# taldatech/soft-intro-vae-pytorch

Hardware: AMD Instinct MI355X
Metric: training images/sec (whole node) at 256x256 bs128 (higher is better)
Workload: dtype f32; 1 GPU; soft_intro_vae celeb256 256x256 zdim=512 channels=[64, 128, 256, 512, 512, 512], full E-step + D-step iteration; global_batch=128, per_gpu_batch=128, parallelism=dp1, decoder_forward_reuse=True, hip_graph=False, batchnorm=local

## Files before the change

### soft-intro-vae-pytorch_amd/csrc/bn.hip

```cpp
#include "common.h"

namespace {

struct SlicePlan {
  int S;
  long long len;
};
static SlicePlan plan_slices(long long n_per_ch, int C) {
  SlicePlan p;
  long long s1 = (n_per_ch + 8191) / 8192;
  long long s2 = 2048 / C;
  if (s2 < 1) s2 = 1;
  long long S = s1 < s2 ? s1 : s2;
  if (S < 1) S = 1;
  long long len = (n_per_ch + S - 1) / S;
  len = (len + 3) & ~3LL;
  p.S = (int)((n_per_ch + len - 1) / len);
  p.len = len;
  return p;
}

}

__device__ __forceinline__ unsigned sign_nibble(const float4 v) {
// ... 54 lines not shown
                                                         float* __restrict__ mean_out,
                                                         float* __restrict__ invstd_out) {
  const int c = blockIdx.x * 64 + threadIdx.x;
  if (c == 0 && num_batches_tracked) *num_batches_tracked += 1;
  if (c >= C) return;
  double sum = 0.0, sq = 0.0;
  for (int s = 0; s < S; ++s) {
    const size_t o = ((size_t)c * S + s) * 2;
    sum += part[o];
    sq += part[o + 1];
  }
  const double mean = sum / count;
  double var = sq / count - mean * mean;
  if (var < 0.0) var = 0.0;
  const float invstd = (float)(1.0 / sqrt(var + (double)eps));
  mean_out[c] = (float)mean;
  invstd_out[c] = invstd;
  if (running_mean) {
    const double unbiased = count > 1.0 ? var * count / (count - 1.0) : var;
    running_mean[c] = (float)((1.0 - momentum) * running_mean[c] + momentum * mean);
    running_var[c] = (float)((1.0 - momentum) * running_var[c] + momentum * unbiased);
  }
}

template <int NT>
__global__ void __launch_bounds__(NT) bn_finalize_conv_kernel(const float* __restrict__ part, int S, int C,
                                                               double count, float eps, float momentum,
                                                               float* running_mean, float* running_var,
                                                               long long* num_batches_tracked,
                                                               float* __restrict__ mean_out,
                                                               float* __restrict__ invstd_out, int nseg, int seg_rev) {
  __shared__ double red[NT / 64];
  const int c = blockIdx.x;
  for (int gi = 0; gi < nseg; ++gi) {
    const int g = seg_rev ? nseg - 1 - gi : gi;
    double sum = 0.0, sq = 0.0;
    for (int s = threadIdx.x; s < S; s += NT) {
      const float2 v = *reinterpret_cast<const float2*>(part + ((size_t)(g * S + s) * C + c) * 2);
      sum += (double)v.x;
      sq += (double)v.y;
    }
    sum = block_sum<NT>(sum, red);
    sq = block_sum<NT>(sq, red);
    if (threadIdx.x == 0) {
      if (c == 0 && num_batches_tracked) *num_batches_tracked += 1;
      const double mean = sum / count;
      double var = sq / count - mean * mean;
      if (var < 0.0) var = 0.0;
      mean_out[g * C + c] = (float)mean;
      invstd_out[g * C + c] = (float)(1.0 / sqrt(var + (double)eps));
      if (running_mean) {
        const double unbiased = count > 1.0 ? var * count / (count - 1.0) : var;
        running_mean[c] = (float)((1.0 - momentum) * running_mean[c] + momentum * mean);
        running_var[c] = (float)((1.0 - momentum) * running_var[c] + momentum * unbiased);
      }
    }
    __syncthreads();
  }
}

extern "C" size_t sivae_bn_workspace_bytes(int B, int C, int HW) {
  if (B <= 0 || C <= 0 || HW <= 0) return 0;
  SlicePlan p = plan_slices((long long)B * HW, C);
  return ((size_t)C * p.S * 2 + (size_t)C * 2) * sizeof(double);
}

extern "C" int sivae_bn_stats(const float* x, int B, int C, int HW, float eps, float momentum,
                              float* running_mean, float* running_var, long long* num_batches_tracked,
                              float* mean_out, float* invstd_out, void* workspace, size_t workspace_bytes,
                              hipStream_t stream) {
  if (!x || !mean_out || !invstd_out) return SIVAE_ERR_NULL;
  if ((running_mean == nullptr) != (running_var == nullptr)) return SIVAE_ERR_NULL;
  if (B <= 0 || C <= 0 || HW <= 0) return SIVAE_ERR_SHAPE;
  if (!workspace || workspace_bytes < sivae_bn_workspace_bytes(B, C, HW)) return SIVAE_ERR_WORKSPACE;
  const long long n = (long long)B * HW;
  SlicePlan p = plan_slices(n, C);
  double* part = (double*)workspace;
  hipLaunchKernelGGL(bn_stats_partial_kernel, dim3(C, p.S), dim3(256), 0, stream, x, part, C, HW, n, p.len, p.S);
  hipLaunchKernelGGL(bn_finalize_kernel, dim3(cdiv(C, 64)), dim3(64), 0, stream, (const double*)part, p.S, C,
                     (double)n, eps, momentum, running_mean, running_var, num_batches_tracked, mean_out,
                     invstd_out);
  return sivae_launch_status();
}

static int bn_stats_from_conv_impl(const float* partials, int n_tiles, int nseg, int seg_rev, int B, int C, int HW,
                                   float eps, float momentum, float* running_mean, float* running_var,
                                   long long* num_batches_tracked, float* mean_out, float* invstd_out,
                                   hipStream_t stream) {
  if (!partials || !mean_out || !invstd_out) return SIVAE_ERR_NULL;
  if ((running_mean == nullptr) != (running_var == nullptr)) return SIVAE_ERR_NULL;
  if (B <= 0 || C <= 0 || HW <= 0 || n_tiles <= 0 || nseg <= 0 || (n_tiles % nseg) != 0) return SIVAE_ERR_SHAPE;
  const int S = n_tiles / nseg;
  if (S >= 4096)
    hipLaunchKernelGGL((bn_finalize_conv_kernel<1024>), dim3(C), dim3(1024), 0, stream, partials, S, C,
                       (double)B * HW, eps, momentum, running_mean, running_var, num_batches_tracked, mean_out,
                       invstd_out, nseg, seg_rev);
  else
    hipLaunchKernelGGL((bn_finalize_conv_kernel<256>), dim3(C), dim3(256), 0, stream, partials, S, C,
                       (double)B * HW, eps, momentum, running_mean, running_var, num_batches_tracked, mean_out,
                       invstd_out, nseg, seg_rev);
  return sivae_launch_status();
}

#define BNC_ROWS 128
__global__ void __launch_bounds__(256) bn_conv_rows_partial_kernel(const float* __restrict__ part, int S, int C,
                                                                   int nchunks, double* __restrict__ out) {
  __shared__ double red[2][256];
  const int chunk = blockIdx.x, g = blockIdx.y, t = threadIdx.x;
  int cw = 1;
  while (cw < C && cw < 256) cw <<= 1;
  const int rp = 256 / cw, tx = t & (cw - 1), ty = t / cw;
  const int r0 = chunk * BNC_ROWS;
  const int r1 = r0 + BNC_ROWS < S ? r0 + BNC_ROWS : S;
  for (int c0 = 0; c0 < C; c0 += cw) {
    const int c = c0 + tx;
    double sum = 0.0, sq = 0.0;
    if (c < C)
      for (int r = r0 + ty; r < r1; r += rp) {
        const float2 v = *reinterpret_cast<const float2*>(part + ((size_t)(g * S + r) * C + c) * 2);
        sum += (double)v.x;
        sq += (double)v.y;
      }
    red[0][t] = sum;
    red[1][t] = sq;
    __syncthreads();
    if (ty == 0 && c < C) {
      double a = 0.0, b = 0.0;
      for (int k = 0; k < rp; ++k) {
        a += red[0][k * cw + tx];
        b += red[1][k * cw + tx];
      }
      double* o = out + (((size_t)g * C + c) * nchunks + chunk) * 2;
      o[0] = a;
      o[1] = b;
    }
    __syncthreads();
  }
}

__global__ void __launch_bounds__(64) bn_conv_rows_finalize_kernel(const double* __restrict__ part2, int nchunks, int C,
                                                                   double count, float eps, float momentum,
                                                                   float* running_mean, float* running_var,
                                                                   long long* num_batches_tracked,
                                                                   float* __restrict__ mean_out,
                                                                   float* __restrict__ invstd_out, int nseg,
                                                                   int seg_rev) {
  const int c = blockIdx.x, lane = threadIdx.x;
  if (c == 0 && lane == 0 && num_batches_tracked) *num_batches_tracked += nseg;
  for (int gi = 0; gi < nseg; ++gi) {
    const int g = seg_rev ? nseg - 1 - gi : gi;
    const double* p = part2 + ((size_t)g * C + c) * nchunks * 2;
    double sum = 0.0, sq = 0.0;
    for (int k = lane; k < nchunks; k += 64) {
      sum += p[2 * k];
      sq += p[2 * k + 1];
    }
    sum = wave_sum(sum);
    sq = wave_sum(sq);
    if (lane == 0) {
      const double mean = sum / count;
      double var = sq / count - mean * mean;
      if (var < 0.0) var = 0.0;
      mean_out[g * C + c] = (float)mean;
      invstd_out[g * C + c] = (float)(1.0 / sqrt(var + (double)eps));
      if (running_mean) {
        const double unbiased = count > 1.0 ? var * count / (count - 1.0) : var;
        running_mean[c] = (float)((1.0 - momentum) * running_mean[c] + momentum * mean);
        running_var[c] = (float)((1.0 - momentum) * running_var[c] + momentum * unbiased);
      }
    }
  }
}

extern "C" size_t sivae_bn_stats_from_conv_workspace_bytes(int n_tiles, int nseg, int C) {
  if (n_tiles <= 0 || nseg <= 0 || C <= 0 || (n_tiles % nseg) != 0) return 0;
  const int S = n_tiles / nseg;
  if (S < 2048) return 0;
  return (size_t)nseg * C * cdiv(S, BNC_ROWS) * 2 * sizeof(double);
}

extern "C" int sivae_bn_stats_from_conv_ws(const float* partials, int n_tiles, int nseg, int seg_rev, int B_seg, int C,
                                           int HW, float eps, float momentum, float* running_mean, float* running_var,
                                           long long* num_batches_tracked, float* mean_out, float* invstd_out,
                                           void* workspace, size_t workspace_bytes, hipStream_t stream) {
  const size_t need = sivae_bn_stats_from_conv_workspace_bytes(n_tiles, nseg, C);
  if (need == 0)
    return bn_stats_from_conv_impl(partials, n_tiles, nseg, seg_rev, B_seg, C, HW, eps, momentum, running_mean,
                                   running_var, num_batches_tracked, mean_out, invstd_out, stream);
  if (!partials || !mean_out || !invstd_out) return SIVAE_ERR_NULL;
  if ((running_mean == nullptr) != (running_var == nullptr)) return SIVAE_ERR_NULL;
  if (B_seg <= 0 || HW <= 0) return SIVAE_ERR_SHAPE;
  if (!workspace || workspace_bytes < need) return SIVAE_ERR_WORKSPACE;
  const int S = n_tiles / nseg, nchunks = cdiv(S, BNC_ROWS);
  double* part2 = (double*)workspace;
  hipLaunchKernelGGL(bn_conv_rows_partial_kernel, dim3(nchunks, nseg), dim3(256), 0, stream, partials, S, C, nchunks,
                     part2);
  hipLaunchKernelGGL(bn_conv_rows_finalize_kernel, dim3(C), dim3(64), 0, stream, (const double*)part2, nchunks,
                     C, (double)B_seg * HW, eps, momentum, running_mean, running_var, num_batches_tracked, mean_out,
                     invstd_out, nseg, seg_rev);
  return sivae_launch_status();
}

extern "C" int sivae_bn_stats_from_conv_seg(const float* partials, int n_tiles, int nseg, int seg_rev, int B_seg, int C,
                                            int HW, float eps, float momentum, float* running_mean, float* running_var,
                                            long long* num_batches_tracked, float* mean_out, float* invstd_out,
                                            hipStream_t stream) {
  return bn_stats_from_conv_impl(partials, n_tiles, nseg, seg_rev, B_seg, C, HW, eps, momentum, running_mean,
                                 running_var, num_batches_tracked, mean_out, invstd_out, stream);
}

__global__ void __launch_bounds__(256) bn_sums_conv_kernel(const float* __restrict__ part, int S, int C,
                                                           double* __restrict__ sums) {
  __shared__ double red[4];
  const int c = blockIdx.x;
  double sum = 0.0, sq = 0.0;
  for (int s = threadIdx.x; s < S; s += 256) {
    const float2 v = *reinterpret_cast<const float2*>(part + ((size_t)s * C + c) * 2);
    sum += (double)v.x;
    sq += (double)v.y;
  }
  sum = block_sum<256>(sum, red);
  sq = block_sum<256>(sq, red);
  if (threadIdx.x == 0) {
    sums[c * 2 + 0] = sum;
    sums[c * 2 + 1] = sq;
  }
}

__global__ void __launch_bounds__(64) bn_finalize_sums_kernel(const double* __restrict__ sums, int C, double count,
                                                              float eps, float momentum, float* running_mean,
                                                              float* running_var, long long* num_batches_tracked,
                                                              float* __restrict__ mean_out,
                                                              float* __restrict__ invstd_out) {
  const int c = blockIdx.x * 64 + threadIdx.x;
  if (c >= C) return;
  if (c == 0 && num_batches_tracked) *num_batches_tracked += 1;
  const double mean = sums[c * 2] / count;
  double var = sums[c * 2 + 1] / count - mean * mean;
  if (var < 0.0) var = 0.0;
  mean_out[c] = (float)mean;
  invstd_out[c] = (float)(1.0 / sqrt(var + (double)eps));
  if (running_mean) {
    const double unbiased = count > 1.0 ? var * count / (count - 1.0) : var;
    running_mean[c] = (float)((1.0 - momentum) * running_mean[c] + momentum * mean);
    running_var[c] = (float)((1.0 - momentum) * running_var[c] + momentum * unbiased);
  }
}

extern "C" int sivae_bn_sums_from_conv(const float* partials, int n_tiles, int C, double* sums, hipStream_t stream) {
  if (!partials || !sums) return SIVAE_ERR_NULL;
  if (C <= 0 || n_tiles <= 0) return SIVAE_ERR_SHAPE;
  hipLaunchKernelGGL(bn_sums_conv_kernel, dim3(C), dim3(256), 0, stream, partials, n_tiles, C, sums);
  return sivae_launch_status();
}

extern "C" int sivae_bn_finalize_sums(const double* sums, int C, double count, float eps, float momentum,
                                      float* running_mean, float* running_var, long long* num_batches_tracked,
                                      float* mean_out, float* invstd_out, hipStream_t stream) {
  if (!sums || !mean_out || !invstd_out) return SIVAE_ERR_NULL;
  if ((running_mean == nullptr) != (running_var == nullptr)) return SIVAE_ERR_NULL;
  if (C <= 0 || !(count > 0.0)) return SIVAE_ERR_SHAPE;
  hipLaunchKernelGGL(bn_finalize_sums_kernel, dim3(cdiv(C, 64)), dim3(64), 0, stream, sums, C, count, eps, momentum,
                     running_mean, running_var, num_batches_tracked, mean_out, invstd_out);
  return sivae_launch_status();
}

__global__ void __launch_bounds__(64) bn_update_running_seg_kernel(const float* __restrict__ mean,
                                                                   const float* __restrict__ invstd, int nseg,
                                                                   int seg_rev, int C, double count, float eps,
                                                                   float momentum, float* running_mean,
                                                                   float* running_var, long long* num_batches_tracked) {
  const int c = blockIdx.x * 64 + threadIdx.x;
  if (c == 0 && num_batches_tracked) *num_batches_tracked += nseg;
  if (c >= C) return;
  float rm = running_mean[c], rv = running_var[c];
  for (int gi = 0; gi < nseg; ++gi) {
    const int g = seg_rev ? nseg - 1 - gi : gi;
    const double is = (double)invstd[g * C + c];
    double var = 1.0 / (is * is) - (double)eps;
    if (var < 0.0) var = 0.0;
    const double unbiased = count > 1.0 ? var * count / (count - 1.0) : var;
    rm = (float)((1.0 - momentum) * rm + momentum * (double)mean[g * C + c]);
    rv = (float)((1.0 - momentum) * rv + momentum * unbiased);
  }
  running_mean[c] = rm;
  running_var[c] = rv;
}

extern "C" int sivae_bn_update_running_seg(const float* mean, const float* invstd, int nseg, int seg_rev, int C,
                                           double count, float eps, float momentum, float* running_mean,
                                           float* running_var, long long* num_batches_tracked, hipStream_t stream) {
  if (!mean || !invstd || !running_mean || !running_var) return SIVAE_ERR_NULL;
  if (C <= 0 || nseg <= 0 || count <= 0.0) return SIVAE_ERR_SHAPE;
  hipLaunchKernelGGL(bn_update_running_seg_kernel, dim3(cdiv(C, 64)), dim3(64), 0, stream, mean, invstd, nseg, seg_rev,
                     C, count, eps, momentum, running_mean, running_var, num_batches_tracked);
  return sivae_launch_status();
}

static bool normalise_segments(int B, int& segB) {
  if (segB < 0 || (segB > 0 && B % segB != 0)) return false;
  if (segB == B) segB = 0;
  return true;
}

template <bool HAS_RES, bool VEC>
__global__ void __launch_bounds__(256) bn_apply_kernel(const float* __restrict__ x, const float* __restrict__ res,
                                                       const float* __restrict__ mean,
                                                       const float* __restrict__ invstd,
                                                       const float* __restrict__ gamma,
                                                       const float* __restrict__ beta, float slope,
                                                       float* __restrict__ y, unsigned char* __restrict__ mask,
                                                       int C, int HW, size_t numel, int segB) {
  const size_t stride = (size_t)gridDim.x * 256;
  if (VEC) {
    const size_t n4 = numel >> 2;
    for (size_t base = (size_t)blockIdx.x * 256; base < n4; base += stride) {
      const size_t i = base + threadIdx.x;
      const bool ok = i < n4;
      unsigned nib = 0;
      if (ok) {
        const size_t e = i << 2;
        const unsigned pl = (unsigned)(e / HW);
        const int c = (int)(pl % (unsigned)C);
        const int sc = segB > 0 ? c + (int)((pl / (unsigned)C) / (unsigned)segB) * C : c;
        const float m = mean[sc], g = invstd[sc] * gamma[c], bt = beta[c];
        float4 v = reinterpret_cast<const float4*>(x)[i];
        v.x = (v.x - m) * g + bt;
        v.y = (v.y - m) * g + bt;
        v.z = (v.z - m) * g + bt;
        v.w = (v.w - m) * g + bt;
        if (HAS_RES) {
          const float4 r = reinterpret_cast<const float4*>(res)[i];
          v.x += r.x; v.y += r.y; v.z += r.z; v.w += r.w;
        }
        nib = sign_nibble(v);
        v.x = lrelu(v.x, slope); v.y = lrelu(v.y, slope); v.z = lrelu(v.z, slope); v.w = lrelu(v.w, slope);
        reinterpret_cast<float4*>(y)[i] = v;
      }
      if (mask != nullptr) {
        const unsigned byte = pair_nibbles(nib);
        if (ok && !(threadIdx.x & 1)) mask[i >> 1] = (unsigned char)byte;
      }
    }
  } else {
    for (size_t e = (size_t)blockIdx.x * 256 + threadIdx.x; e < numel; e += stride) {
      const unsigned pl = (unsigned)(e / HW);
      const int c = (int)(pl % (unsigned)C);
      const int sc = segB > 0 ? c + (int)((pl / (unsigned)C) / (unsigned)segB) * C : c;
      float v = (x[e] - mean[sc]) * (invstd[sc] * gamma[c]) + beta[c];
      if (HAS_RES) v += res[e];
      y[e] = lrelu(v, slope);
    }
  }
}

static int bn_apply_impl(const float* x, const float* res, const float* mean, const float* invstd,
                         const float* gamma, const float* beta, float slope, float* y, unsigned char* mask, int B,
                         int C, int HW, hipStream_t stream, int segB) {
  if (!x || !mean || !invstd || !gamma || !beta || !y) return SIVAE_ERR_NULL;
  if (B <= 0 || C <= 0 || HW <= 0) return SIVAE_ERR_SHAPE;
  if (!normalise_segments(B, segB)) return SIVAE_ERR_SHAPE;
  const size_t numel = (size_t)B * C * HW;
  const bool vec = (HW & 3) == 0;
  if (mask && !vec) return SIVAE_ERR_SHAPE;
  long long work = vec ? (long long)(numel >> 2) : (long long)numel;
  int nb = cdiv(work, 256);
  if (nb > 8192) nb = 8192;
  if (nb < 1) nb = 1;
#define LAUNCH(R, V) \
  hipLaunchKernelGGL((bn_apply_kernel<R, V>), dim3(nb), dim3(256), 0, stream, x, res, mean, invstd, gamma, beta, \
                     slope, y, mask, C, HW, numel, segB)
  if (res) {
    if (vec) LAUNCH(true, true); else LAUNCH(true, false);
  } else {
    if (vec) LAUNCH(false, true); else LAUNCH(false, false);
  }
#undef LAUNCH
  return sivae_launch_status();
}

__global__ void __launch_bounds__(256) bn_apply_resup_kernel(const float* __restrict__ x, const float* __restrict__ res,
                                                             const float* __restrict__ mean,
                                                             const float* __restrict__ invstd,
                                                             const float* __restrict__ gamma,
                                                             const float* __restrict__ beta, float slope,
                                                             float* __restrict__ y, unsigned char* __restrict__ mask,
                                                             int C, int H, int W, size_t numel, int segB) {
  const size_t stride = (size_t)gridDim.x * 256;
  const int W4 = W >> 2, Hs = H >> 1, Ws = W >> 1;
  const size_t n4 = numel >> 2;
  for (size_t base = (size_t)blockIdx.x * 256; base < n4; base += stride) {
    const size_t i = base + threadIdx.x;
    const bool ok = i < n4;
    unsigned nib = 0;
    if (ok) {
      const int w4 = (int)(i % W4);
      size_t t = i / W4;
      const int h = (int)(t % H);
      t /= H;
      const int c = (int)(t % C);
      const int sc = segB > 0 ? c + (int)(((unsigned)t / (unsigned)C) / (unsigned)segB) * C : c;
      const float m = mean[sc], g = invstd[sc] * gamma[c], bt = beta[c];
      float4 v = reinterpret_cast<const float4*>(x)[i];
      const float2 r = *reinterpret_cast<const float2*>(res + (t * Hs + (h >> 1)) * Ws + 2 * w4);
      v.x = (v.x - m) * g + bt + r.x;
      v.y = (v.y - m) * g + bt + r.x;
      v.z = (v.z - m) * g + bt + r.y;
      v.w = (v.w - m) * g + bt + r.y;
      nib = sign_nibble(v);
      v.x = lrelu(v.x, slope); v.y = lrelu(v.y, slope); v.z = lrelu(v.z, slope); v.w = lrelu(v.w, slope);
      reinterpret_cast<float4*>(y)[i] = v;
    }
    if (mask != nullptr) {
      const unsigned byte = pair_nibbles(nib);
      if (ok && !(threadIdx.x & 1)) mask[i >> 1] = (unsigned char)byte;
    }
  }
}

static int bn_apply_resup_impl(const float* x, const float* res_half, const float* mean, const float* invstd,
                               const float* gamma, const float* beta, float slope, float* y, unsigned char* mask,
                               int B, int C, int H, int W, hipStream_t stream, int segB) {
  if (!x || !res_half || !mean || !invstd || !gamma || !beta || !y) return SIVAE_ERR_NULL;
  if (B <= 0 || C <= 0 || H <= 0 || W <= 0 || (H & 1) || (W & 3)) return SIVAE_ERR_SHAPE;
  if (!normalise_segments(B, segB)) return SIVAE_ERR_SHAPE;
  const size_t numel = (size_t)B * C * H * W;
  int nb = cdiv((long long)(numel >> 2), 256 * 4);
  if (nb > 8192) nb = 8192;
  if (nb < 1) nb = 1;
  hipLaunchKernelGGL(bn_apply_resup_kernel, dim3(nb), dim3(256), 0, stream, x, res_half, mean, invstd, gamma, beta,
                     slope, y, mask, C, H, W, numel, segB);
  return sivae_launch_status();
}

template <bool HAS_RES>
__global__ void __launch_bounds__(256) bn_apply_pool_kernel(const float* __restrict__ x, const float* __restrict__ res,
                                                            const float* __restrict__ mean,
                                                            const float* __restrict__ invstd,
                                                            const float* __restrict__ gamma,
                                                            const float* __restrict__ beta, float slope,
                                                            float* __restrict__ y, float* __restrict__ yp,
                                                            unsigned char* __restrict__ mask, int C, int H, int W,
                                                            size_t n_quads, int segB) {
  const size_t stride = (size_t)gridDim.x * 256;
  const int W4 = W >> 2, H2 = H >> 1;
  for (size_t base = (size_t)blockIdx.x * 256; base < n_quads; base += stride) {
    const size_t i = base + threadIdx.x;
    const bool ok = i < n_quads;
    unsigned nib0 = 0, nib1 = 0;
    size_t m0 = 0, m1 = 0;
    if (ok) {
      const int w4 = (int)(i % W4);
      size_t t = i / W4;
      const int h2 = (int)(t % H2);
      t /= H2;
      const int c = (int)(t % C);
      const int sc = segB > 0 ? c + (int)(((unsigned)t / (unsigned)C) / (unsigned)segB) * C : c;
      const float m = mean[sc], g = invstd[sc] * gamma[c], bt = beta[c];
      const size_t o0 = (t * H + 2 * h2) * (size_t)W + 4 * w4, o1 = o0 + W;
      float4 a = *reinterpret_cast<const float4*>(x + o0), b = *reinterpret_cast<const float4*>(x + o1);
      a.x = (a.x - m) * g + bt; a.y = (a.y - m) * g + bt; a.z = (a.z - m) * g + bt; a.w = (a.w - m) * g + bt;
      b.x = (b.x - m) * g + bt; b.y = (b.y - m) * g + bt; b.z = (b.z - m) * g + bt; b.w = (b.w - m) * g + bt;
      if (HAS_RES) {
        const float4 ra = *reinterpret_cast<const float4*>(res + o0), rb = *reinterpret_cast<const float4*>(res + o1);
        a.x += ra.x; a.y += ra.y; a.z += ra.z; a.w += ra.w;
        b.x += rb.x; b.y += rb.y; b.z += rb.z; b.w += rb.w;
      }
      nib0 = sign_nibble(a);
      nib1 = sign_nibble(b);
      m0 = o0 >> 3;
      m1 = o1 >> 3;
      a.x = lrelu(a.x, slope); a.y = lrelu(a.y, slope); a.z = lrelu(a.z, slope); a.w = lrelu(a.w, slope);
      b.x = lrelu(b.x, slope); b.y = lrelu(b.y, slope); b.z = lrelu(b.z, slope); b.w = lrelu(b.w, slope);
      if (y != nullptr) {
        *reinterpret_cast<float4*>(y + o0) = a;
        *reinterpret_cast<float4*>(y + o1) = b;
      }
      *reinterpret_cast<float2*>(yp + (t * H2 + h2) * (size_t)(W >> 1) + 2 * w4) =
          make_float2(((a.x + a.y) + (b.x + b.y)) * 0.25f, ((a.z + a.w) + (b.z + b.w)) * 0.25f);
    }
    if (mask != nullptr) {
      const unsigned byte0 = pair_nibbles(nib0), byte1 = pair_nibbles(nib1);
      if (ok && !(threadIdx.x & 1)) {
        mask[m0] = (unsigned char)byte0;
        mask[m1] = (unsigned char)byte1;
      }
    }
  }
}

static int bn_apply_pool_impl(const float* x, const float* res, const float* mean, const float* invstd,
                              const float* gamma, const float* beta, float slope, float* y, float* y_pooled,
                              unsigned char* mask, int B, int C, int H, int W, hipStream_t stream, int segB) {
  if (!x || !mean || !invstd || !gamma || !beta || !y_pooled) return SIVAE_ERR_NULL;
  if (B <= 0 || C <= 0 || H <= 0 || W <= 0 || (H & 1) || (W & 3)) return SIVAE_ERR_SHAPE;
  if (!normalise_segments(B, segB)) return SIVAE_ERR_SHAPE;
  if (mask && (W & 7)) return SIVAE_ERR_SHAPE;
  const size_t n_quads = (size_t)B * C * (H >> 1) * (W >> 2);
  int nb = cdiv((long long)n_quads, 256 * 2);
  if (nb > 8192) nb = 8192;
  if (nb < 1) nb = 1;
  if (res)
    hipLaunchKernelGGL(bn_apply_pool_kernel<true>, dim3(nb), dim3(256), 0, stream, x, res, mean, invstd, gamma, beta,
                       slope, y, y_pooled, mask, C, H, W, n_quads, segB);
  else
    hipLaunchKernelGGL(bn_apply_pool_kernel<false>, dim3(nb), dim3(256), 0, stream, x, res, mean, invstd, gamma, beta,
                       slope, y, y_pooled, mask, C, H, W, n_quads, segB);
  return sivae_launch_status();
}

static int bn_apply_any(const float* x, const float* res, int res_up, const float* mean, const float* invstd,
                        const float* gamma, const float* beta, float slope, float* y, float* y_pooled,
                        unsigned char* mask, int B, int C, int H, int W, int segB, hipStream_t stream) {
  if (y_pooled) {
    if (res_up) return SIVAE_ERR_MODE;
    return bn_apply_pool_impl(x, res, mean, invstd, gamma, beta, slope, y, y_pooled, mask, B, C, H, W, stream, segB);
  }
  if (res_up) return bn_apply_resup_impl(x, res, mean, invstd, gamma, beta, slope, y, mask, B, C, H, W, stream, segB);
  return bn_apply_impl(x, res, mean, invstd, gamma, beta, slope, y, mask, B, C, H * W, stream, segB);
}

extern "C" int sivae_bn_apply_act_seg(const float* x, const float* res, int res_up, const float* mean,
                                      const float* invstd, const float* gamma, const float* beta, float slope,
                                      float* y, float* y_pooled, int B, int C, int H, int W, int seg_images,
                                      hipStream_t stream) {
  if (seg_images <= 0) return SIVAE_ERR_SHAPE;
  return bn_apply_any(x, res, res_up, mean, invstd, gamma, beta, slope, y, y_pooled, nullptr, B, C, H, W, seg_images,
                      stream);
}

extern "C" size_t sivae_bn_signmask_bytes(int B, int C, int HW) {
  if (B <= 0 || C <= 0 || HW <= 0) return 0;
  return ((size_t)B * C * HW + 7) / 8;
}

extern "C" int sivae_bn_apply_act_signmask_seg(const float* x, const float* res, int res_up, const float* mean,
                                               const float* invstd, const float* gamma, const float* beta, float slope,
                                               float* y, float* y_pooled, unsigned char* mask, int B, int C, int H,
                                               int W, int seg_images, hipStream_t stream) {
  if (seg_images <= 0) return SIVAE_ERR_SHAPE;
  if (!mask) return SIVAE_ERR_NULL;
  if (H <= 0 || W <= 0 || (H & 1) || (W & 7)) return SIVAE_ERR_SHAPE;
  return bn_apply_any(x, res, res_up, mean, invstd, gamma, beta, slope, y, y_pooled, mask, B, C, H, W, seg_images,
                      stream);
}

__device__ __forceinline__ float4 bn_load_dy4(const float* __restrict__ dy, size_t pl, int hw, int HW, int pool_w) {
  if (pool_w == 0) return *reinterpret_cast<const float4*>(dy + pl * HW + hw);
  const int h = hw / pool_w, w = hw - h * pool_w;
  const float2 d = *reinterpret_cast<const float2*>(dy + pl * (size_t)(HW >> 2) + (size_t)(h >> 1) * (pool_w >> 1) + (w >> 1));
  return make_float4(0.25f * d.x, 0.25f * d.x, 0.25f * d.y, 0.25f * d.y);
}

template <int ACT>
__global__ void __launch_bounds__(256) bn_bwd_partial_kernel(const float* __restrict__ dy, const float* __restrict__ y,
                                                             const float* __restrict__ x,
                                                             const float* __restrict__ mean,
                                                             const float* __restrict__ invstd,
                                                             const float* __restrict__ gamma,
                                                             const float* __restrict__ beta, float slope,
                                                             double* __restrict__ part, int C, int HW,
                                                             long long n_per_ch, long long slice_len, int S,
                                                             int pool_w, const unsigned char* __restrict__ mask,
                                                             int segB, unsigned* __restrict__ counters, int nseg,
                                                             double count, float* __restrict__ dgamma,
                                                             float* __restrict__ dbeta, float* __restrict__ coef) {
  __shared__ double red[4];
  __shared__ int is_last;
  const int vc = blockIdx.x, s = blockIdx.y;
  const int c = vc % C;
  const long long b0 = (long long)(vc / C) * segB;
  const long long n0 = (long long)s * slice_len;
  long long n1 = n0 + slice_len;
  if (n1 > n_per_ch) n1 = n_per_ch;
  const float m = mean[vc], is = invstd[vc];
  const float gsc = ACT == 2 ? is * gamma[c] : 0.f, bt = ACT == 2 ? beta[c] : 0.f;
  double s1 = 0.0, s2 = 0.0;
  if ((HW & 3) == 0) {
    for (long long n = n0 + (long long)threadIdx.x * 4; n < n1; n += 1024) {
      const long long bl = n / HW, b = bl + b0;
      const size_t o = ((size_t)b * C + c) * HW + (size_t)(n - bl * HW);
      const float4 g = bn_load_dy4(dy, (size_t)b * C + c, (int)(n - bl * HW), HW, pool_w);
      const float4 xv = *reinterpret_cast<const float4*>(x + o);
      float gz[4] = {g.x, g.y, g.z, g.w};
      if (ACT == 1) {
        const float4 yv = *reinterpret_cast<const float4*>(y + o);
        gz[0] = yv.x > 0.f ? gz[0] : gz[0] * slope;
        gz[1] = yv.y > 0.f ? gz[1] : gz[1] * slope;
        gz[2] = yv.z > 0.f ? gz[2] : gz[2] * slope;
        gz[3] = yv.w > 0.f ? gz[3] : gz[3] * slope;
      } else if (ACT == 2) {
        gz[0] = ((xv.x - m) * gsc + bt) > 0.f ? gz[0] : gz[0] * slope;
        gz[1] = ((xv.y - m) * gsc + bt) > 0.f ? gz[1] : gz[1] * slope;
        gz[2] = ((xv.z - m) * gsc + bt) > 0.f ? gz[2] : gz[2] * slope;
        gz[3] = ((xv.w - m) * gsc + bt) > 0.f ? gz[3] : gz[3] * slope;
      } else if (ACT == 3) {
        apply_nibble(gz, load_nibble(mask, o >> 2), slope);
      }
      const float xh[4] = {(xv.x - m) * is, (xv.y - m) * is, (xv.z - m) * is, (xv.w - m) * is};
#pragma unroll
      for (int k = 0; k < 4; ++k) {
        s1 += (double)gz[k];
        s2 += (double)gz[k] * (double)xh[k];
      }
    }
  } else {
    for (long long n = n0 + threadIdx.x; n < n1; n += 256) {
      const long long bl = n / HW, b = bl + b0;
      const size_t o = ((size_t)b * C + c) * HW + (size_t)(n - bl * HW);
      float g = dy[o];
      if (ACT == 1) g = y[o] > 0.f ? g : g * slope;
      if (ACT == 2) g = ((x[o] - m) * gsc + bt) > 0.f ? g : g * slope;
      s1 += (double)g;
      s2 += (double)g * (double)((x[o] - m) * is);
    }
  }
  s1 = block_sum<256>(s1, red);
  s2 = block_sum<256>(s2, red);
  if (threadIdx.x == 0) {
    part[((size_t)vc * S + s) * 2 + 0] = s1;
    part[((size_t)vc * S + s) * 2 + 1] = s2;
  }
  if (counters == nullptr) return;
  if (threadIdx.x == 0) {
    __threadfence();
    const unsigned done = atomicAdd(&counters[c], 1u);
    is_last = done == (unsigned)(nseg * S) - 1u;
  }
  __syncthreads();
  if (is_last && threadIdx.x == 0) {
    __threadfence();
    double t1 = 0.0, t2 = 0.0;
    for (int g = 0; g < nseg; ++g) {
      const int v = g * C + c;
      double a1 = 0.0, a2 = 0.0;
      for (int k = 0; k < S; ++k) {
        a1 += __hip_atomic_load(&part[((size_t)v * S + k) * 2 + 0], __ATOMIC_RELAXED, __HIP_MEMORY_SCOPE_AGENT);
        a2 += __hip_atomic_load(&part[((size_t)v * S + k) * 2 + 1], __ATOMIC_RELAXED, __HIP_MEMORY_SCOPE_AGENT);
      }
      coef[v * 2 + 0] = (float)(a1 / count);
      coef[v * 2 + 1] = (float)(a2 / count);
      t1 += a1;
      t2 += a2;
    }
    if (dbeta) dbeta[c] = (float)t1;
    if (dgamma) dgamma[c] = (float)t2;
    counters[c] = 0u;
  }
}

__global__ void __launch_bounds__(64) bn_bwd_finalize_kernel(const double* __restrict__ part, int S, int C,
                                                             double count, float* __restrict__ dgamma,
                                                             float* __restrict__ dbeta, float* __restrict__ coef,
                                                             int nseg) {
  const int c = blockIdx.x * 64 + threadIdx.x;
  if (c >= C) return;
  double t1 = 0.0, t2 = 0.0;
  for (int g = 0; g < nseg; ++g) {
    const int vc = g * C + c;
    double s1 = 0.0, s2 = 0.0;
    for (int s = 0; s < S; ++s) {
      s1 += part[((size_t)vc * S + s) * 2 + 0];
      s2 += part[((size_t)vc * S + s) * 2 + 1];
    }
    coef[vc * 2 + 0] = (float)(s1 / count);
    coef[vc * 2 + 1] = (float)(s2 / count);
    t1 += s1;
    t2 += s2;
  }
  if (dbeta) dbeta[c] = (float)t1;
  if (dgamma) dgamma[c] = (float)t2;
}

template <int ACT, bool HAS_DZ, bool VEC>
__global__ void __launch_bounds__(256) bn_bwd_dx_kernel(const float* __restrict__ dy, const float* __restrict__ y,
                                                        const float* __restrict__ x, const float* __restrict__ mean,
                                                        const float* __restrict__ invstd,
                                                        const float* __restrict__ gamma,
                                                        const float* __restrict__ beta,
                                                        const float* __restrict__ coef, float slope,
                                                        float* __restrict__ dx, float* __restrict__ dz_out, int C,
                                                        int HW, size_t numel, int pool_w,
                                                        const unsigned char* __restrict__ mask, int segB) {
  const size_t stride = (size_t)gridDim.x * 256;
  if (VEC) {
    const size_t n4 = numel >> 2;
    for (size_t i = (size_t)blockIdx.x * 256 + threadIdx.x; i < n4; i += stride) {
      const size_t e = i << 2;
      const unsigned pl = (unsigned)(e / HW);
      const int c = (int)(pl % (unsigned)C);
      const int sc = segB > 0 ? c + (int)((pl / (unsigned)C) / (unsigned)segB) * C : c;
      const float m = mean[sc], is = invstd[sc], gs = gamma[c] * is, c1 = coef[sc * 2], c2 = coef[sc * 2 + 1];
      const float4 g = bn_load_dy4(dy, e / HW, (int)(e % HW), HW, pool_w);
      const float4 xv = reinterpret_cast<const float4*>(x)[i];
      float gz[4] = {g.x, g.y, g.z, g.w};
      if (ACT == 1) {
        const float4 yv = reinterpret_cast<const float4*>(y)[i];
        gz[0] = yv.x > 0.f ? gz[0] : gz[0] * slope;
        gz[1] = yv.y > 0.f ? gz[1] : gz[1] * slope;
        gz[2] = yv.z > 0.f ? gz[2] : gz[2] * slope;
        gz[3] = yv.w > 0.f ? gz[3] : gz[3] * slope;
      } else if (ACT == 2) {
        const float bt = beta[c];
        gz[0] = ((xv.x - m) * gs + bt) > 0.f ? gz[0] : gz[0] * slope;
        gz[1] = ((xv.y - m) * gs + bt) > 0.f ? gz[1] : gz[1] * slope;
        gz[2] = ((xv.z - m) * gs + bt) > 0.f ? gz[2] : gz[2] * slope;
        gz[3] = ((xv.w - m) * gs + bt) > 0.f ? gz[3] : gz[3] * slope;
      } else if (ACT == 3) {
        apply_nibble(gz, load_nibble(mask, i), slope);
      }
      float4 o;
      o.x = gs * (gz[0] - c1 - (xv.x - m) * is * c2);
      o.y = gs * (gz[1] - c1 - (xv.y - m) * is * c2);
      o.z = gs * (gz[2] - c1 - (xv.z - m) * is * c2);
      o.w = gs * (gz[3] - c1 - (xv.w - m) * is * c2);
      reinterpret_cast<float4*>(dx)[i] = o;
      if (HAS_DZ) reinterpret_cast<float4*>(dz_out)[i] = make_float4(gz[0], gz[1], gz[2], gz[3]);
    }
  } else {
    for (size_t e = (size_t)blockIdx.x * 256 + threadIdx.x; e < numel; e += stride) {
      const unsigned pl = (unsigned)(e / HW);
      const int c = (int)(pl % (unsigned)C);
      const int sc = segB > 0 ? c + (int)((pl / (unsigned)C) / (unsigned)segB) * C : c;
      const float m = mean[sc], is = invstd[sc];
      float g = dy[e];
      if (ACT == 1) g = y[e] > 0.f ? g : g * slope;
      if (ACT == 2) g = ((x[e] - m) * (is * gamma[c]) + beta[c]) > 0.f ? g : g * slope;
      dx[e] = gamma[c] * is * (g - coef[sc * 2] - (x[e] - m) * is * coef[sc * 2 + 1]);
      if (HAS_DZ) dz_out[e] = g;
    }
  }
}

template <bool MASK>
__global__ void __launch_bounds__(256) bn_bwd_dx_dzsum_kernel(const float* __restrict__ dy, const float* __restrict__ y,
                                                              const float* __restrict__ x,
                                                              const float* __restrict__ mean,
                                                              const float* __restrict__ invstd,
                                                              const float* __restrict__ gamma,
                                                              const float* __restrict__ coef, float slope,
                                                              float* __restrict__ dx, float* __restrict__ dz_half, int C,
                                                              int H, int W, size_t n_quads,
                                                              const unsigned char* __restrict__ mask, int segB) {
  const size_t stride = (size_t)gridDim.x * 256;
  const int W4 = W >> 2, H2 = H >> 1;
  for (size_t i = (size_t)blockIdx.x * 256 + threadIdx.x; i < n_quads; i += stride) {
    const int w4 = (int)(i % W4);
    size_t t = i / W4;
    const int h2 = (int)(t % H2);
    t /= H2;
    const int c = (int)(t % C);
    const int sc = segB > 0 ? c + (int)(((unsigned)t / (unsigned)C) / (unsigned)segB) * C : c;
    const float m = mean[sc], is = invstd[sc], gs = gamma[c] * is, c1 = coef[sc * 2], c2 = coef[sc * 2 + 1];
    const size_t o0 = (t * H + 2 * h2) * (size_t)W + 4 * w4;
    float gsum[2] = {0.f, 0.f};
    float row0[2] = {0.f, 0.f};
#pragma unroll
    for (int rr = 0; rr < 2; ++rr) {
      const size_t o = o0 + (size_t)rr * W;
      const float4 g = *reinterpret_cast<const float4*>(dy + o);
      const float4 xv = *reinterpret_cast<const float4*>(x + o);
      float gzv[4] = {g.x, g.y, g.z, g.w};
      if (MASK) {
        apply_nibble(gzv, load_nibble(mask, o >> 2), slope);
      } else {
        const float4 yv = *reinterpret_cast<const float4*>(y + o);
        gzv[0] = yv.x > 0.f ? g.x : g.x * slope; gzv[1] = yv.y > 0.f ? g.y : g.y * slope;
        gzv[2] = yv.z > 0.f ? g.z : g.z * slope; gzv[3] = yv.w > 0.f ? g.w : g.w * slope;
      }
      const float gz0 = gzv[0], gz1 = gzv[1], gz2 = gzv[2], gz3 = gzv[3];
      float4 d;
      d.x = gs * (gz0 - c1 - (xv.x - m) * is * c2);
      d.y = gs * (gz1 - c1 - (xv.y - m) * is * c2);
      d.z = gs * (gz2 - c1 - (xv.z - m) * is * c2);
      d.w = gs * (gz3 - c1 - (xv.w - m) * is * c2);
      *reinterpret_cast<float4*>(dx + o) = d;
      if (rr == 0) {
        row0[0] = gz0 + gz1;
        row0[1] = gz2 + gz3;
      } else {
        gsum[0] = row0[0] + (gz0 + gz1);
        gsum[1] = row0[1] + (gz2 + gz3);
      }
    }
    *reinterpret_cast<float2*>(dz_half + (t * H2 + h2) * (size_t)(W >> 1) + 2 * w4) = make_float2(gsum[0], gsum[1]);
  }
}

static int bn_bwd_impl(const float* dy, const float* y, const float* x, const float* mean, const float* invstd,
                       const float* gamma, const float* beta, int act_mode, float slope, float* dx, float* dz_out,
                       float* dgamma, float* dbeta, int B, int C, int HW, int pool_w, void* workspace,
                       size_t workspace_bytes, hipStream_t stream, int dzsum_w, const unsigned char* mask,
                       int segB, unsigned* counters) {
  if (!dy || !x || !mean || !invstd || !gamma || !dx) return SIVAE_ERR_NULL;
  if (act_mode < 0 || act_mode > 3) return SIVAE_ERR_MODE;
  if (act_mode == 1 && !y) return SIVAE_ERR_NULL;
  if (act_mode == 3 && (!mask || (HW & 3))) return SIVAE_ERR_NULL;
  if (act_mode == 2 && !beta) return SIVAE_ERR_NULL;
  if (B <= 0 || C <= 0 || HW <= 0) return SIVAE_ERR_SHAPE;
  if (!normalise_segments(B, segB)) return SIVAE_ERR_SHAPE;
  const int nseg = segB > 0 ? B / segB : 1, Bs = segB > 0 ? segB : B, VC = nseg * C;
  const long long n = (long long)Bs * HW;
  SlicePlan p = plan_slices(n, VC);
  if (!workspace || workspace_bytes < ((size_t)VC * p.S * 2 + (size_t)VC * 2) * sizeof(double)) return SIVAE_ERR_WORKSPACE;
  double* part = (double*)workspace;
  float* coef = (float*)(part + (size_t)VC * p.S * 2);
#define LAUNCHP(A) \
  hipLaunchKernelGGL((bn_bwd_partial_kernel<A>), dim3(VC, p.S), dim3(256), 0, stream, dy, y, x, mean, invstd, gamma, \
                     beta, slope, part, C, HW, n, p.len, p.S, pool_w, mask, Bs, counters, nseg, (double)n, dgamma, \
                     dbeta, coef)
  if (act_mode == 0) LAUNCHP(0); else if (act_mode == 1) LAUNCHP(1); else if (act_mode == 2) LAUNCHP(2); else LAUNCHP(3);
// ... 205 lines not shown
```

Measured before the change: 340.0 img/s.

## Add per-plane streaming BN-apply kernels with hoisted per-channel coefficients

Adds new batchnorm-apply kernels that launch a 3D grid over (span, channel, batch), so each block works on one contiguous plane. The per-channel mean, invstd, gamma and beta are loaded once per block instead of being recomputed from a per-element channel index with division and modulo. Loads are batched before the compute under a scheduling barrier to raise memory-level parallelism. Covers the plain, residual-upsample and fused-pool variants when HW is at least 512, and can be turned off with an environment variable; small planes still use the old grid-stride kernels.

```diff
diff --git a/soft-intro-vae-pytorch_amd/csrc/bn.hip b/soft-intro-vae-pytorch_amd/csrc/bn.hip
--- a/soft-intro-vae-pytorch_amd/csrc/bn.hip
+++ b/soft-intro-vae-pytorch_amd/csrc/bn.hip
@@ -380,6 +380,15 @@
   if (segB == B) segB = 0;
   return true;
 }
+
+static bool bn_apply_stream_wanted(int B, int C, long long HW);
+static void bn_apply_stream_launch(const float* x, const float* res, const float* mean, const float* invstd,
+                                   const float* gamma, const float* beta, float slope, float* y, unsigned char* mask,
+                                   int B, int C, int HW, hipStream_t stream, int segB);
+static void bn_apply_stream_quad_launch(const float* x, const float* res, int res_up, const float* mean,
+                                        const float* invstd, const float* gamma, const float* beta, float slope,
+                                        float* y, float* y_pooled, unsigned char* mask, int B, int C, int H, int W,
+                                        hipStream_t stream, int segB);
 
 template <bool HAS_RES, bool VEC>
 __global__ void __launch_bounds__(256) bn_apply_kernel(const float* __restrict__ x, const float* __restrict__ res,
@@ -441,6 +450,10 @@
   const size_t numel = (size_t)B * C * HW;
   const bool vec = (HW & 3) == 0;
   if (mask && !vec) return SIVAE_ERR_SHAPE;
+  if (vec && (!mask || (HW & 7) == 0) && bn_apply_stream_wanted(B, C, HW)) {
+    bn_apply_stream_launch(x, res, mean, invstd, gamma, beta, slope, y, mask, B, C, HW, stream, segB);
+    return sivae_launch_status();
+  }
   long long work = vec ? (long long)(numel >> 2) : (long long)numel;
   int nb = cdiv(work, 256);
   if (nb > 8192) nb = 8192;
@@ -502,6 +515,11 @@
   if (!x || !res_half || !mean || !invstd || !gamma || !beta || !y) return SIVAE_ERR_NULL;
   if (B <= 0 || C <= 0 || H <= 0 || W <= 0 || (H & 1) || (W & 3)) return SIVAE_ERR_SHAPE;
   if (!normalise_segments(B, segB)) return SIVAE_ERR_SHAPE;
+  if ((!mask || (W & 7) == 0) && bn_apply_stream_wanted(B, C, (long long)H * W)) {
+    bn_apply_stream_quad_launch(x, res_half, 1, mean, invstd, gamma, beta, slope, y, nullptr, mask, B, C, H, W, stream,
+                                segB);
+    return sivae_launch_status();
+  }
   const size_t numel = (size_t)B * C * H * W;
   int nb = cdiv((long long)(numel >> 2), 256 * 4);
   if (nb > 8192) nb = 8192;
@@ -574,6 +592,10 @@
   if (B <= 0 || C <= 0 || H <= 0 || W <= 0 || (H & 1) || (W & 3)) return SIVAE_ERR_SHAPE;
   if (!normalise_segments(B, segB)) return SIVAE_ERR_SHAPE;
   if (mask && (W & 7)) return SIVAE_ERR_SHAPE;
+  if (bn_apply_stream_wanted(B, C, (long long)H * W)) {
+    bn_apply_stream_quad_launch(x, res, 0, mean, invstd, gamma, beta, slope, y, y_pooled, mask, B, C, H, W, stream, segB);
+    return sivae_launch_status();
+  }
   const size_t n_quads = (size_t)B * C * (H >> 1) * (W >> 2);
   int nb = cdiv((long long)n_quads, 256 * 2);
   if (nb > 8192) nb = 8192;
@@ -585,6 +607,248 @@
     hipLaunchKernelGGL(bn_apply_pool_kernel<false>, dim3(nb), dim3(256), 0, stream, x, res, mean, invstd, gamma, beta,
                        slope, y, y_pooled, mask, C, H, W, n_quads, segB);
   return sivae_launch_status();
+}
+
+#ifndef BNS_MIN_HW
+#define BNS_MIN_HW 512
+#endif
+#define BNS_MAX_HW (1 << 28)
+
+struct BnsCoef {
+  float m, g, bt;
+};
+__device__ __forceinline__ BnsCoef bns_coef(const float* __restrict__ mean, const float* __restrict__ invstd,
+                                            const float* __restrict__ gamma, const float* __restrict__ beta, unsigned c,
+                                            unsigned b, int C, int segB) {
+  const unsigned sc = segB > 0 ? c + (b / (unsigned)segB) * (unsigned)C : c;
+  BnsCoef k;
+  k.m = mean[sc];
+  k.g = invstd[sc] * gamma[c];
+  k.bt = beta[c];
+  return k;
+}
+__device__ __forceinline__ float4 bns_ld4(const char* p, unsigned off) { return *reinterpret_cast<const float4*>(p + off); }
+__device__ __forceinline__ float2 bns_ld2(const char* p, unsigned off) { return *reinterpret_cast<const float2*>(p + off); }
+__device__ __forceinline__ void bns_st4(char* p, unsigned off, const float4 v) { *reinterpret_cast<float4*>(p + off) = v; }
+__device__ __forceinline__ void bns_st2(char* p, unsigned off, const float2 v) { *reinterpret_cast<float2*>(p + off) = v; }
+
+template <bool HAS_RES, bool MASK, bool GUARD>
+__device__ __forceinline__ void bns_plain_tile(const char* __restrict__ xp, const char* __restrict__ rp,
+                                               char* __restrict__ yp, unsigned char* __restrict__ mp, unsigned o,
+                                               unsigned end, const BnsCoef k, float slope) {
+  const float m = k.m, g = k.g, bt = k.bt;
+  float4 v[4], r[4];
+  bool ok[4];
+#pragma unroll
+  for (int u = 0; u < 4; ++u) {
+    const unsigned i = o + u * 256;
+    ok[u] = !GUARD || i < end;
+    v[u] = make_float4(0.f, 0.f, 0.f, 0.f);
+    r[u] = v[u];
+    if (ok[u]) {
+      v[u] = bns_ld4(xp, i << 4);
+      if (HAS_RES) r[u] = bns_ld4(rp, i << 4);
+    }
+  }
+  __builtin_amdgcn_sched_barrier(0);
+#pragma unroll
+  for (int u = 0; u < 4; ++u) {
+    const unsigned i = o + u * 256;
+    unsigned nib = 0;
+    if (ok[u]) {
+      float4 w = v[u];
+      w.x = (w.x - m) * g + bt;
+      w.y = (w.y - m) * g + bt;
+      w.z = (w.z - m) * g + bt;
+      w.w = (w.w - m) * g + bt;
+      if (HAS_RES) {
+        w.x += r[u].x; w.y += r[u].y; w.z += r[u].z; w.w += r[u].w;
+      }
+      nib = sign_nibble(w);
+      w.x = lrelu(w.x, slope); w.y = lrelu(w.y, slope); w.z = lrelu(w.z, slope); w.w = lrelu(w.w, slope);
+      bns_st4(yp, i << 4, w);
+    }
+    if (MASK) {
+      const unsigned byte = pair_nibbles(nib);
+      if (ok[u] && !(threadIdx.x & 1)) mp[i >> 1] = (unsigned char)byte;
+    }
+  }
+}
+
+template <bool HAS_RES, bool MASK>
+__global__ void __launch_bounds__(256) bn_apply_stream_kernel(const float* __restrict__ x, const float* __restrict__ res,
+                                                              const float* __restrict__ mean,
+                                                              const float* __restrict__ invstd,
+                                                              const float* __restrict__ gamma,
+                                                              const float* __restrict__ beta, float slope,
+                                                              float* __restrict__ y, unsigned char* __restrict__ mask,
+                                                              int C, unsigned n4, unsigned span, int segB) {
+  const unsigned c = blockIdx.y, b = blockIdx.z;
+  const BnsCoef k = bns_coef(mean, invstd, gamma, beta, c, b, C, segB);
+  const size_t plane = (size_t)b * C + c;
+  const char* xp = reinterpret_cast<const char*>(x + plane * n4 * 4);
+  const char* rp = HAS_RES ? reinterpret_cast<const char*>(res + plane * n4 * 4) : nullptr;
+  char* yp = reinterpret_cast<char*>(y + plane * n4 * 4);
+  unsigned char* mp = MASK ? mask + plane * (n4 >> 1) : nullptr;
+  const unsigned s0 = blockIdx.x * span;
+  const unsigned s1 = s0 + span < n4 ? s0 + span : n4;
+  unsigned base = s0;
+  for (; base + 1024 <= s1; base += 1024)
+    bns_plain_tile<HAS_RES, MASK, false>(xp, rp, yp, mp, base + threadIdx.x, s1, k, slope);
+  if (base < s1) bns_plain_tile<HAS_RES, MASK, true>(xp, rp, yp, mp, base + threadIdx.x, s1, k, slope);
+}
+
+template <int MODE, bool HAS_RES, bool HAS_Y, bool MASK, bool GUARD>
+__device__ __forceinline__ void bns_quad_tile(const char* __restrict__ xp, const char* __restrict__ rp,
+                                              char* __restrict__ yp, char* __restrict__ pp,
+                                              unsigned char* __restrict__ mp, unsigned q, unsigned& w4, unsigned W4,
+                                              unsigned wstep, unsigned end, const BnsCoef k, float slope) {
+  const float m = k.m, g = k.g, bt = k.bt;
+  float4 a[2], b[2], ra[2], rb[2];
+  float2 rh[2];
+  unsigned oa[2];
+  bool ok[2];
+#pragma unroll
+  for (int u = 0; u < 2; ++u) {
+    const unsigned qu = q + u * 256;
+    ok[u] = !GUARD || qu < end;
+    oa[u] = 2 * qu - w4;
+    w4 += wstep;
+    if (w4 >= W4) w4 -= W4;
+    a[u] = make_float4(0.f, 0.f, 0.f, 0.f);
+    b[u] = ra[u] = rb[u] = a[u];
+    rh[u] = make_float2(0.f, 0.f);
+    if (ok[u]) {
+      a[u] = bns_ld4(xp, oa[u] << 4);
+      b[u] = bns_ld4(xp, (oa[u] + W4) << 4);
+      if (MODE == 1) rh[u] = bns_ld2(rp, qu << 3);
+      if (MODE == 2 && HAS_RES) {
+        ra[u] = bns_ld4(rp, oa[u] << 4);
+        rb[u] = bns_ld4(rp, (oa[u] + W4) << 4);
+      }
+    }
+  }
+  __builtin_amdgcn_sched_barrier(0);
+#pragma unroll
+  for (int u = 0; u < 2; ++u) {
+    const unsigned qu = q + u * 256;
+    unsigned nib0 = 0, nib1 = 0;
+    if (ok[u]) {
+      float4 va = a[u], vb = b[u];
+      if (MODE == 1) {
+        const float2 r = rh[u];
+        va.x = (va.x - m) * g + bt + r.x;
+        va.y = (va.y - m) * g + bt + r.x;
+        va.z = (va.z - m) * g + bt + r.y;
+        va.w = (va.w - m) * g + bt + r.y;
+        vb.x = (vb.x - m) * g + bt + r.x;
+        vb.y = (vb.y - m) * g + bt + r.x;
+        vb.z = (vb.z - m) * g + bt + r.y;
+        vb.w = (vb.w - m) * g + bt + r.y;
+      } else {
+        va.x = (va.x - m) * g + bt; va.y = (va.y - m) * g + bt; va.z = (va.z - m) * g + bt; va.w = (va.w - m) * g + bt;
+        vb.x = (vb.x - m) * g + bt; vb.y = (vb.y - m) * g + bt; vb.z = (vb.z - m) * g + bt; vb.w = (vb.w - m) * g + bt;
+        if (HAS_RES) {
+          va.x += ra[u].x; va.y += ra[u].y; va.z += ra[u].z; va.w += ra[u].w;
+          vb.x += rb[u].x; vb.y += rb[u].y; vb.z += rb[u].z; vb.w += rb[u].w;
+        }
+      }
+      nib0 = sign_nibble(va);
+      nib1 = sign_nibble(vb);
+      va.x = lrelu(va.x, slope); va.y = lrelu(va.y, slope); va.z = lrelu(va.z, slope); va.w = lrelu(va.w, slope);
+      vb.x = lrelu(vb.x, slope); vb.y = lrelu(vb.y, slope); vb.z = lrelu(vb.z, slope); vb.w = lrelu(vb.w, slope);
+      if (HAS_Y) {
+        bns_st4(yp, oa[u] << 4, va);
+        bns_st4(yp, (oa[u] + W4) << 4, vb);
+      }
+      if (MODE == 2)
+        bns_st2(pp, qu << 3,
+                make_float2(((va.x + va.y) + (vb.x + vb.y)) * 0.25f, ((va.z + va.w) + (vb.z + vb.w)) * 0.25f));
+    }
+    if (MASK) {
+      const unsigned byte0 = pair_nibbles(nib0), byte1 = pair_nibbles(nib1);
+      if (ok[u] && !(threadIdx.x & 1)) {
+        mp[oa[u] >> 1] = (unsigned char)byte0;
+        mp[(oa[u] + W4) >> 1] = (unsigned char)byte1;
+      }
+    }
+  }
+}
+
+template <int MODE, bool HAS_RES, bool HAS_Y, bool MASK>
+__global__ void __launch_bounds__(256) bn_apply_stream_quad_kernel(const float* __restrict__ x,
+                                                                   const float* __restrict__ res,
+                                                                   const float* __restrict__ mean,
+                                                                   const float* __restrict__ invstd,
+                                                                   const float* __restrict__ gamma,
+                                                                   const float* __restrict__ beta, float slope,
+                                                                   float* __restrict__ y, float* __restrict__ yp_out,
+                                                                   unsigned char* __restrict__ mask, int C, unsigned nq,
+                                                                   unsigned W4, unsigned wstep, unsigned span,
+                                                                   int segB) {
+  const unsigned c = blockIdx.y, b = blockIdx.z;
+  const BnsCoef k = bns_coef(mean, invstd, gamma, beta, c, b, C, segB);
+  const size_t plane = (size_t)b * C + c;
+  const char* xp = reinterpret_cast<const char*>(x + plane * nq * 8);
+  const char* rp = !HAS_RES ? nullptr : reinterpret_cast<const char*>(res + plane * nq * (MODE == 1 ? 2 : 8));
+  char* yp = HAS_Y ? reinterpret_cast<char*>(y + plane * nq * 8) : nullptr;
+  char* pp = MODE == 2 ? reinterpret_cast<char*>(yp_out + plane * nq * 2) : nullptr;
+  unsigned char* mp = MASK ? mask + plane * nq : nullptr;
+  const unsigned s0 = blockIdx.x * span;
+  const unsigned s1 = s0 + span < nq ? s0 + span : nq;
+  unsigned w4 = (s0 + threadIdx.x) % W4;
+  unsigned base = s0;
+  for (; base + 512 <= s1; base += 512)
+    bns_quad_tile<MODE, HAS_RES, HAS_Y, MASK, false>(xp, rp, yp, pp, mp, base + threadIdx.x, w4, W4, wstep, s1, k, slope);
+  if (base < s1)
+    bns_quad_tile<MODE, HAS_RES, HAS_Y, MASK, true>(xp, rp, yp, pp, mp, base + threadIdx.x, w4, W4, wstep, s1, k, slope);
+}
+
+static bool bn_apply_stream_wanted(int B, int C, long long HW) {
+  const char* e = getenv("SIVAE_BN_APPLY_STREAM");
+  if (e && e[0] == '0') return false;
+  return HW >= BNS_MIN_HW && HW <= BNS_MAX_HW && (HW & 3) == 0 && B <= 65535 && C <= 65535;
+}
+
+static unsigned bns_span(unsigned tile) { return 2 * tile; }
+
+static void bn_apply_stream_launch(const float* x, const float* res, const float* mean, const float* invstd,
+                                   const float* gamma, const float* beta, float slope, float* y, unsigned char* mask,
+                                   int B, int C, int HW, hipStream_t stream, int segB) {
+  const unsigned n4 = (unsigned)HW >> 2, span = bns_span(1024);
+  const dim3 grid(cdiv(n4, span), C, B);
+#define LAUNCH(R, M) \
+  hipLaunchKernelGGL((bn_apply_stream_kernel<R, M>), grid, dim3(256), 0, stream, x, res, mean, invstd, gamma, beta, \
+                     slope, y, mask, C, n4, span, segB)
+  if (res) {
+    if (mask) LAUNCH(true, true); else LAUNCH(true, false);
+  } else {
+    if (mask) LAUNCH(false, true); else LAUNCH(false, false);
+  }
+#undef LAUNCH
+}
+
+static void bn_apply_stream_quad_launch(const float* x, const float* res, int res_up, const float* mean,
+                                        const float* invstd, const float* gamma, const float* beta, float slope,
+                                        float* y, float* y_pooled, unsigned char* mask, int B, int C, int H, int W,
+                                        hipStream_t stream, int segB) {
+  const unsigned W4 = (unsigned)W >> 2, nq = (unsigned)(H >> 1) * W4, span = bns_span(512);
+  const unsigned wstep = 256u % W4;
+  const dim3 grid(cdiv(nq, span), C, B);
+#define LAUNCH(MODE, R, Y, M) \
+  hipLaunchKernelGGL((bn_apply_stream_quad_kernel<MODE, R, Y, M>), grid, dim3(256), 0, stream, x, res, mean, invstd, \
+                     gamma, beta, slope, y, y_pooled, mask, C, nq, W4, wstep, span, segB)
+#define LAUNCH_M(MODE, R, Y) \
+  do { if (mask) LAUNCH(MODE, R, Y, true); else LAUNCH(MODE, R, Y, false); } while (0)
+  if (res_up) {
+    LAUNCH_M(1, true, true);
+  } else if (res) {
+    if (y) LAUNCH_M(2, true, true); else LAUNCH_M(2, true, false);
+  } else {
+    if (y) LAUNCH_M(2, false, true); else LAUNCH_M(2, false, false);
+  }
+#undef LAUNCH_M
+#undef LAUNCH
 }
 
 static int bn_apply_any(const float* x, const float* res, int res_up, const float* mean, const float* invstd,
```

Measured after the change: 341.7 img/s (median of 6 runs). Within noise of the previous version (+0.5%).
